# smoggy-P/gym-Drone2D-ActivePerception

Measured on NVIDIA B200. Metric: env-steps/sec, higher is better.
Workload: dtype f64

## Files before the change

### gym_drone2d_activeperception_b200/csrc/d2d_step.cuh

```cuda
#pragma once
#include "d2d_state.cuh"
#include "d2d_math.cuh"
#include "d2d_agent_math.cuh"

#if defined(D2D_COLD_NOINLINE) && D2D_COLD_NOINLINE
#define D2D_COLD __noinline__
#else
#define D2D_COLD __forceinline__
#endif

__device__ __forceinline__ uint32_t d2d_smem_u32(const void *p) { return (uint32_t)__cvta_generic_to_shared(p); }
__device__ __forceinline__ void d2d_mbar_init(uint64_t *bar, uint32_t count) {
    asm volatile("mbarrier.init.shared::cta.b64 [%0], %1;" ::"r"(d2d_smem_u32(bar)), "r"(count) : "memory");
    asm volatile("fence.mbarrier_init.release.cluster;" ::: "memory");
}
__device__ __forceinline__ void d2d_mbar_expect_tx(uint64_t *bar, uint32_t bytes) {
    asm volatile("mbarrier.arrive.expect_tx.shared::cta.b64 _, [%0], %1;" ::"r"(d2d_smem_u32(bar)), "r"(bytes) : "memory");
}
__device__ __forceinline__ void d2d_bulk_g2s(void *dst_smem, const void *src_gmem, uint32_t bytes, uint64_t *bar) {
    asm volatile("cp.async.bulk.shared::cluster.global.mbarrier::complete_tx::bytes [%0], [%1], %2, [%3];" ::"r"(
                     d2d_smem_u32(dst_smem)),
                 "l"(src_gmem), "r"(bytes), "r"(d2d_smem_u32(bar))
                 : "memory");
}
// ... 201 lines not shown
        double vx = pref.x, vy = pref.y;
        const bool rvo = P.motion_rvo != 0;
        if (rvo) {
            const double2 v = P.avel_next[g];
            P.avel[g] = v;
            vx = v.x; vy = v.y;
        }
        const double nx = pos.x + vx * P.dt, ny = pos.y + vy * P.dt;
        bool rebound = false;
        if (d2d_norm2_le(vx, vy, 5.0)) {
            const double qx = D2D_FMA(C6, pref.x, -S6 * pref.y);
            const double qy = D2D_FMA(S6, pref.x, C6 * pref.y);
            pref.x = qx; pref.y = qy;
            rebound = true;
        }
        const double edge = P.scale;
        if (nx < edge + r) pref.x = fabs(pref.x);
        else if (nx > P.map_w - edge - r) pref.x = -fabs(pref.x);
        if (ny < edge + r) pref.y = fabs(pref.y);
        else if (ny > P.map_h - edge - r) pref.y = -fabs(pref.y);
        if (!rebound && !rvo) { vx = pref.x; vy = pref.y; }
        pos.x = pos.x + vx * P.dt;
        pos.y = pos.y + vy * P.dt;
        P.apos[g] = pos;
        P.apref[g] = pref;
        if (PF && keep_pos && w == tid) { *keep_pos = pos; *keep_pref = pref; }
        const int q = i * NP + k;
        c.sx[q] = pos.x; c.sy[q] = pos.y; c.sr2[q] = r * r;
        const double ddx = pos.x - s.px, ddy = pos.y - s.py;
        const double reach = r + P.cull_reach;
        if (ddx * ddx + ddy * ddy <= reach * reach) {
            const int slot = atomicAdd(&s.ncull, 1);
            c.cull[i * NP + slot] = (uint16_t)k;
        }
        if (COLLIDE_HERE) {
            if (d2d_norm2_lt(ddx, ddy, r + P.drone_r)) atomicOr(&s.coll_agent, 1);
        }
    }
}

struct RayOut {
    uint8_t *bel_s;
    int e;
    int patch;
    int wi, wj;
    int border_ok;
    uint32_t *chg;
    int *nchg;
    int defer_mirror;
};
#define D2D_CHG_CAP 64
#define D2D_ACTION_SENTINEL 0x7FF8D2D0AC710F05ull
#define D2D_FUSED_WARP_EXTRA (D2D_CHG_CAP * 4 + 16)

__device__ __forceinline__ void d2d_mark_store(const DevP &P, const RayOut &o, int cell, uint8_t v) {
    o.bel_s[cell] = v;
#if defined(D2D_WARP_PROF) && D2D_WARP_PROF >= 2
    atomicAdd(&P.prof[(size_t)o.e * 12 + 5], 1ull);
#endif
    P.belief[(size_t)o.e * D2D_BELIEF_STRIDE + cell] = v;
    if (o.patch) {
        const int ci = cell / D2D_GRID, cj = cell - ci * D2D_GRID;
        const int u = ci - o.wi, w = cj - o.wj;
        if ((unsigned)u < (unsigned)D2D_LOCAL && (unsigned)w < (unsigned)D2D_LOCAL) {
            const size_t off = (size_t)o.e * D2D_LOCAL_CELLS + u * D2D_LOCAL + w;
            P.local_map[off] = v;
            if (P.lm_mirror && !o.defer_mirror) {
                P.lm_mirror[off] = v;
                atomicAdd((int *)(o.bel_s + D2D_MIRCNT_OFF), 1);
            }
        }
    }
    if (o.chg) {
        const int slot = atomicAdd(o.nchg, 1);
        if (slot < D2D_CHG_CAP) o.chg[slot] = (uint32_t)cell | ((uint32_t)v << 16);
    }
}
__device__ __forceinline__ void d2d_mark(const DevP &P, const RayOut &o, int ci, int cj, uint8_t v) {
    const int cell = ci * D2D_GRID + cj;
    if (o.bel_s[cell] != v) d2d_mark_store(P, o, cell, v);
}

__device__ __forceinline__ double d2d_ray_angle(const DevP &P, double yaw, int ray) {
    const double ray_angle = P.ray_a0 + P.ray_da * (double)ray;
    const double player_angle = D2D_TWO_PI - yaw * D2D_DEG2RAD;
    double a = player_angle + ray_angle;
    a = copysign(d2d_pymod(fabs(a), D2D_TWO_PI), a);
    if (a < 0) a += D2D_TWO_PI;
    return a;
}

template <bool SAFE = false, bool SMALL = false>
__device__ __forceinline__ uint32_t d2d_cast_ray(const DevP &P, const EnvS &s, double a, double slope, const RayOut &o,
                                                 const uint64_t *gt, const double *sx, const double *sy, const double *sr2,
                                                 const uint16_t *cull, uint32_t *hitw) {
    uint32_t hm = 0u;
    const bool faced_right = (a < 90.0 * D2D_DEG2RAD) || (a > 270.0 * D2D_DEG2RAD);
    const bool faced_up = a > D2D_PI;
    const double step = P.scale - 1.0;
    double xs, ys;
    if (fabs(slope) > 1.0) {
        slope = 1.0 / slope;
        ys = faced_up ? -step : step;
        xs = ys * slope;
    } else {
        xs = faced_right ? step : -step;
        ys = xs * slope;
    }
    const double x0 = s.px, y0 = s.py;
    const int nc = s.ncull;
    uint32_t cmask = 0u;
    int mlo = 0x7fff, mhi = -1;
    {
        const double dd2 = xs * xs + ys * ys;
        const float inv_dd2 = 1.0f / (float)dd2;
        const int ncm = (SMALL || nc < 32) ? nc : 32;
#pragma unroll 1
        for (int q = 0; q < ncm; q++) {
            const int k = cull[q];
            const double cx = sx[k] - x0, cy = sy[k] - y0;
            const double cr = cx * ys - cy * xs;
            const double rr = sr2[k] * 1.000001 + 1e-3;
            if (cr * cr <= rr * dd2) {
                cmask |= 1u << q;
                const float t = (float)(cx * xs + cy * ys) * inv_dd2;
                const float hw = sqrtf((float)rr * inv_dd2) + 0.05f;
                mlo = min(mlo, (int)ceilf(t - hw));
                mhi = max(mhi, (int)floorf(t + hw));
            }
        }
        if (!SMALL && nc > 32) { mlo = 0; mhi = 0x7fff; }
    }
    const unsigned mspan = mhi >= mlo ? (unsigned)(mhi - mlo) : 0u;
    if (SAFE) {
        const bool xup = xs > 0.0, yup = ys > 0.0;
        int dcx = xup ? D2D_GRID : -D2D_GRID, dcy = yup ? 1 : -1;
        asm volatile("" : "+r"(dcx), "+r"(dcy));
        const double uxs = fabs(xs), uys = fabs(ys);
        const double ux0 = xup ? x0 : -x0, uy0 = yup ? y0 : -y0;
        double ux = ux0, uy = uy0;
        double uxb = xup ? P.scale * (double)(s.ix + 1) : -(P.scale * (double)s.ix);
        double uyb = yup ? P.scale * (double)(s.iy + 1) : -(P.scale * (double)s.iy);
        const double scale = P.scale;
        const uint32_t bel0 = d2d_smem_u32(o.bel_s);
        uint32_t caddr = bel0 + (uint32_t)(s.ix * D2D_GRID + s.iy);
        int m = 0;
        for (;;) {
            if ((unsigned)(m - mlo) <= mspan) {
                const double x = dcx > 0 ? ux : -ux, y = dcy > 0 ? uy : -uy;
                if (!(0.0 < x && 0.0 < y)) break;
                bool any = false;
                uint32_t mm = cmask;
                while (mm) {
                    const int q = __ffs(mm) - 1;
                    mm &= mm - 1u;
                    const int k = cull[q];
                    const double ex = sx[k] - x, ey = sy[k] - y;
                    if (ex * ex + ey * ey <= sr2[k]) { hm |= 1u << q; any = true; }
                }
                if (!SMALL) {
#pragma unroll 1
                    for (int q = 32; q < nc; q++) {
                        const int k = cull[q];
                        const double ex = sx[k] - x, ey = sy[k] - y;
                        if (ex * ex + ey * ey <= sr2[k]) { atomicOr(&hitw[k >> 5], 1u << (k & 31)); any = true; }
                    }
                }
                if (any) break;
            }
            uint32_t bel;
            asm volatile("ld.shared.u8 %0, [%1];" : "=r"(bel) : "r"(caddr));
            if (bel != 2u) {
                if (bel == 1u) break;
                const int cell = (int)(caddr - bel0);
                const int ci = cell / D2D_GRID, cj = cell - ci * D2D_GRID;
                if ((gt[ci] >> cj) & 1ull) {
                    bool in_map = true;
                    if (ci == 0 || cj == 0) {
                        const double x = dcx > 0 ? ux : -ux, y = dcy > 0 ? uy : -uy;
                        in_map = 0.0 < x && 0.0 < y;
                    }
                    if (in_map) d2d_mark_store(P, o, cell, 1);
                    break;
                }
                if (m >= P.m_far) {
                    const double fx = ux - ux0, fy = uy - uy0;
                    if ((fx * fx + fy * fy) >= P.depth2) break;
                }
                d2d_mark_store(P, o, cell, 2);
            } else if (m >= P.m_far) {
                const double fx = ux - ux0, fy = uy - uy0;
                if ((fx * fx + fy * fy) >= P.depth2) break;
            }
            m += 1;
            asm("{\n\t"
                ".reg .pred pe, pn;\n\t"
                "add.rn.f64 %0, %0, %3;\n\t"
                "setp.lt.s32 pn, %4, 0;\n\t"
                "setp.eq.and.f64 pe, %0, %1, pn;\n\t"
                "setp.lt.or.f64 pe, %0, %1, pe;\n\t"
                "@!pe add.s32 %2, %2, %4;\n\t"
                "@!pe add.rn.f64 %1, %1, %5;\n\t"
                "}" : "+d"(ux), "+d"(uxb), "+r"(caddr) : "d"(uxs), "r"(dcx), "d"(scale));
            asm("{\n\t"
                ".reg .pred pe, pn;\n\t"
                "add.rn.f64 %0, %0, %3;\n\t"
                "setp.lt.s32 pn, %4, 0;\n\t"
                "setp.eq.and.f64 pe, %0, %1, pn;\n\t"
                "setp.lt.or.f64 pe, %0, %1, pe;\n\t"
                "@!pe add.s32 %2, %2, %4;\n\t"
                "@!pe add.rn.f64 %1, %1, %5;\n\t"
                "}" : "+d"(uy), "+d"(uyb), "+r"(caddr) : "d"(uys), "r"(dcy), "d"(scale));
        }
#if defined(D2D_WARP_PROF) && D2D_WARP_PROF >= 2
        atomicAdd(&P.prof[(size_t)o.e * 12 + 6], (unsigned long long)(m + 1));
        atomicMax(&P.prof[(size_t)o.e * 12 + 7], (unsigned long long)(m + 1));
#endif
        return hm;
    }
    int ci = s.ix, cj = s.iy;
    const bool xup = xs > 0.0, yup = ys > 0.0;
    const int sxi = xup ? 1 : -1, syi = yup ? 1 : -1;
    const double uxs = fabs(xs), uys = fabs(ys);
    double ux = xup ? x0 : -x0, uy = yup ? y0 : -y0;
    double uxb = xup ? P.scale * (double)(ci + 1) : -(P.scale * (double)ci);
    double uyb = yup ? P.scale * (double)(cj + 1) : -(P.scale * (double)cj);
    int m = 0;
    for (;;) {
        if ((unsigned)(ci - 1) >= (unsigned)(D2D_GRID - 2) || (unsigned)(cj - 1) >= (unsigned)(D2D_GRID - 2)) {
            const double x = xup ? ux : -ux, y = yup ? uy : -uy;
            if (!(0.0 < x && x < P.map_w && 0.0 < y && y < P.map_h)) break;
        }
        if ((unsigned)(m - mlo) <= mspan) {
            const double x = xup ? ux : -ux, y = yup ? uy : -uy;
            bool any = false;
            uint32_t mm = cmask;
            while (mm) {
                const int q = __ffs(mm) - 1;
                mm &= mm - 1u;
                const int k = cull[q];
                const double ex = sx[k] - x, ey = sy[k] - y;
                if (ex * ex + ey * ey <= sr2[k]) {
                    hm |= 1u << q;
                    any = true;
                }
            }
            if (!SMALL) {
#pragma unroll 1
                for (int q = 32; q < nc; q++) {
                    const int k = cull[q];
                    const double ex = sx[k] - x, ey = sy[k] - y;
                    if (ex * ex + ey * ey <= sr2[k]) {
                        atomicOr(&hitw[k >> 5], 1u << (k & 31));
                        any = true;
                    }
                }
            }
            if (any) break;
        }
        const bool wall = (gt[ci] >> cj) & 1ull;
        bool far = false;
        if (m >= P.m_far) {
            const double fx = ux - (xup ? x0 : -x0), fy = uy - (yup ? y0 : -y0);
            far = (fx * fx + fy * fy) >= P.depth2;
        }
        if (wall || far) {
            if (wall) d2d_mark(P, o, ci, cj, 1);
            break;
        }
        d2d_mark(P, o, ci, cj, 2);
        ux = ux + uxs;
        uy = uy + uys;
        m += 1;
        bool cx = ux >= uxb, cy = uy >= uyb;
        if (ux == uxb || uy == uyb) {
            if (ux == uxb && !xup) cx = false;
            if (uy == uyb && !yup) cy = false;
        }
        if (cx) { ci += sxi; uxb += P.scale; }
        if (cy) { cj += syi; uyb += P.scale; }
    }
    return hm;
}

__device__ __forceinline__ void d2d_publish_hits(uint32_t hm, const uint16_t *cull, uint32_t *hitw) {
    while (hm) {
        const int q = __ffs(hm) - 1;
        hm &= hm - 1u;
        const int k = cull[q];
        atomicOr(&hitw[k >> 5], 1u << (k & 31));
    }
}

__device__ __forceinline__ void d2d_phase_rays(const DevP &P, const BlockCtx &c, int env0, int E, int tid, int T) {
    const int R = P.n_rays, NP = P.NP;
    for (int w = tid; w < E * R; w += T) {
        const int i = w / R, ray = w - i * R;
        const EnvS &s = c.S[i];
        if (!s.valid) continue;
        RayOut o;
        o.bel_s = c.belief + (size_t)i * D2D_BELIEF_STRIDE;
        o.e = env0 + i; o.patch = 0; o.wi = 0; o.wj = 0; o.border_ok = 0; o.chg = nullptr; o.nchg = nullptr; o.defer_mirror = 0;
        const double a = d2d_ray_angle(P, s.yaw, ray);
        const uint32_t hm = d2d_cast_ray(P, s, a, d2d_tan(a), o, c.gt + (size_t)i * D2D_GRID, c.sx + i * NP, c.sy + i * NP,
                                         c.sr2 + i * NP, c.cull + i * NP, c.hitw + i * P.HW);
        d2d_publish_hits(hm, c.cull + i * NP, c.hitw + i * P.HW);
    }
}

__device__ __forceinline__ int d2d_border_intact(const uint64_t *gt, int lane) {
    const uint64_t FULL = (1ull << D2D_GRID) - 1ull, EDGE = 1ull | (1ull << (D2D_GRID - 1));
    bool ok = true;
#pragma unroll
    for (int r = lane; r < D2D_GRID; r += 32) {
        const uint64_t need = (r == 0 || r == D2D_GRID - 1) ? FULL : EDGE;
        ok = ok && ((gt[r] & need) == need);
    }
    return __all_sync(0xffffffffu, ok) ? 1 : 0;
}

template <bool ILP2, bool SMALL = false>
__device__ __forceinline__ uint32_t d2d_phase_rays_warp(const DevP &P, const BlockCtx &c, const RayOut &o, int lane) {
    static_assert(!(ILP2 && SMALL), "the small-crowd form casts one ray per lane per pass");
    const EnvS &s = c.S[0];
    const int R = P.n_rays;
    uint32_t hm = 0u;
    if (ILP2) {
        for (int r0 = lane; r0 < R; r0 += 64) {
            const int r1 = r0 + 32;
            const double a0 = d2d_ray_angle(P, s.yaw, r0), a1 = d2d_ray_angle(P, s.yaw, r1);
            const double t0 = d2d_tan(a0), t1 = d2d_tan(a1);
            hm |= d2d_cast_ray(P, s, a0, t0, o, c.gt, c.sx, c.sy, c.sr2, c.cull, c.hitw);
            if (r1 < R) hm |= d2d_cast_ray(P, s, a1, t1, o, c.gt, c.sx, c.sy, c.sr2, c.cull, c.hitw);
        }
    } else {
        const bool safe = o.border_ok && (unsigned)s.ix < (unsigned)D2D_GRID && (unsigned)s.iy < (unsigned)D2D_GRID;
#pragma unroll 1
        for (int ray = lane; ray < R; ray += 32) {
            const double a = d2d_ray_angle(P, s.yaw, ray);
            const double tn = d2d_tan(a);
            if (safe) hm |= d2d_cast_ray<true, SMALL>(P, s, a, tn, o, c.gt, c.sx, c.sy, c.sr2, c.cull, c.hitw);
            else hm |= d2d_cast_ray<false, SMALL>(P, s, a, tn, o, c.gt, c.sx, c.sy, c.sr2, c.cull, c.hitw);
        }
    }
    hm = __reduce_or_sync(0xffffffffu, hm);
    if (SMALL) return __reduce_or_sync(0xffffffffu, ((hm >> lane) & 1u) ? 1u << c.cull[lane] : 0u);
    if ((hm >> lane) & 1u) {
        const int k = c.cull[lane];
        atomicOr(&c.hitw[k >> 5], 1u << (k & 31));
    }
    return 0u;
}

struct D2DRng {
    uint32_t *key;
    int pos, has;
    double gauss;
};
__device__ __noinline__ void d2d_mt_regen(uint32_t *mt) {
    const uint32_t UP = 0x80000000u, LO = 0x7fffffffu, MA = 0x9908b0dfu;
    int kk;
    uint32_t y;
#pragma unroll 1
    for (kk = 0; kk < 624 - 397; kk++) { y = (mt[kk] & UP) | (mt[kk + 1] & LO); mt[kk] = mt[kk + 397] ^ (y >> 1) ^ ((y & 1u) ? MA : 0u); }
#pragma unroll 1
    for (; kk < 623; kk++) { y = (mt[kk] & UP) | (mt[kk + 1] & LO); mt[kk] = mt[kk + (397 - 624)] ^ (y >> 1) ^ ((y & 1u) ? MA : 0u); }
    y = (mt[623] & UP) | (mt[0] & LO); mt[623] = mt[396] ^ (y >> 1) ^ ((y & 1u) ? MA : 0u);
}
__device__ __forceinline__ uint32_t d2d_mt_next32(D2DRng &r) {
    if (r.pos == 624) { d2d_mt_regen(r.key); r.pos = 0; }
    uint32_t y = r.key[r.pos++];
    y ^= (y >> 11); y ^= (y << 7) & 0x9d2c5680u; y ^= (y << 15) & 0xefc60000u; y ^= (y >> 18);
    return y;
}
__device__ __forceinline__ double d2d_mt_next_double(D2DRng &r) {
    const int a = (int)(d2d_mt_next32(r) >> 5), b = (int)(d2d_mt_next32(r) >> 6);
    return ((double)a * 67108864.0 + (double)b) / 9007199254740992.0;
}
__device__ __noinline__ double d2d_legacy_gauss(D2DRng &r) {
    if (r.has) { const double t = r.gauss; r.has = 0; r.gauss = 0.0; return t; }
    double f, x1, x2, r2;
    do {
        x1 = 2.0 * d2d_mt_next_double(r) - 1.0;
        x2 = 2.0 * d2d_mt_next_double(r) - 1.0;
        r2 = x1 * x1 + x2 * x2;
    } while (r2 >= 1.0 || r2 == 0.0);
// ... 584 lines not shown
        }
        if (lane == 0) atomicAdd(&P.stats[D2D_STAT_MIRROR_BYTES], (unsigned long long)n_changed);
    }
    if (s.done_now) d2d_count_explored_warp(P, c.belief, lane);
    D2D_PROF(3);
}


__device__ __forceinline__ bool d2d_agents_lane(const DevP &P, const BlockCtx &c, EnvS &s, size_t g, int lane, double2 &pos,
                                                double2 &pref, double r) {
    bool in = false, hit = false;
    if (lane < P.N) {
        d2d_cvm_agent_step(pos.x, pos.y, pref.x, pref.y, r, P.dt, P.scale, P.map_w, P.map_h);
        P.apos[g] = pos;
        P.apref[g] = pref;
        c.sx[lane] = pos.x; c.sy[lane] = pos.y; c.sr2[lane] = r * r;
        const double ddx = pos.x - s.px, ddy = pos.y - s.py;
        const double reach = r + P.cull_reach;
        in = ddx * ddx + ddy * ddy <= reach * reach;
        hit = d2d_norm2_lt(ddx, ddy, r + P.drone_r);
    }
    const uint32_t b = __ballot_sync(0xffffffffu, in);
    if (in) c.cull[__popc(b & ((1u << lane) - 1u))] = (uint16_t)lane;
    if (lane == 0) s.ncull = __popc(b);
    return __any_sync(0xffffffffu, hit);
}

__device__ __forceinline__ void d2d_trackers_lane(const DevP &P, const BlockCtx &c, EnvS &s, size_t g, int lane, uint32_t hmask,
                                                  uint8_t pf_act) {
    if (lane >= P.N) return;
    const bool hit = (hmask >> lane) & 1u;
    P.hit[g] = hit ? 1 : 0;
    if (P.trackers) {
        const bool was_active = !s.reset && pf_act != 0;
        if (hit && !was_active) atomicAdd(&s.newly, 1);
        if (was_active || hit || s.reset) {
            const bool noisy = P.var_cam != 0.0;
            d2d_tracker_update(P, s, g, hit, noisy ? c.mx[lane] : c.sx[lane], noisy ? c.my[lane] : c.sy[lane], was_active);
        }
    }
}

__device__ __forceinline__ void d2d_leader_nomove(const DevP &P, EnvS &s, const uint64_t *gt, int e, double action, bool coll,
                                                  int &inv) {
    const int shit = inv & 1;
    bool goal = (inv & 2) != 0;
    s.tgx = -1.0; s.tgy = -1.0;
    if (s.nseg * P.n_way - s.cursor > 0) {
        d2d_leader_finish(P, s, gt, e, 0.0, true, false);
        s.ix = d2d_cell(s.px, P.scale, P.inv_scale); s.iy = d2d_cell(s.py, P.scale, P.inv_scale);
        goal = d2d_norm2_le(s.px - s.tgx, s.py - s.tgy, 10.0);
        int sh = 0;
        for (int q = 0; q < 5; q++) sh |= d2d_static_probe(P, gt, s.px, s.py, q);
        inv = sh | (goal ? 2 : 0);
    } else {
        s.sm = SM_EXECUTING; s.fail = 0;
    }
    s.yaw = d2d_pymod(s.yaw + (action * P.max_yaw_speed) * P.dt, 360.0);
    const int col = shit ? 1 : (coll ? 2 : 0);
    int frz = 0;
    if (col == 0) {
        if (goal) s.sm = SM_GOAL_REACHED;
        frz = ((double)s.steps >= P.max_steps) ? 1 : 0;
    }
    const int done = (col != 0 || frz || (s.sm == SM_GOAL_REACHED && s.tcur >= P.n_targets)) ? 1 : 0;
    s.bufc += s.arch_cnt; s.bufts += s.arch_ts; s.tracked += s.newly;
    if (done) { s.bufc += s.act_cnt; s.bufts += s.act_ts; }
    s.done_now = done;
    P.collision[e] = (uint8_t)col; P.dead_lock[e] = 0; P.freezing[e] = (uint8_t)frz; P.done[e] = (uint8_t)done;
    P.yaw_obs[e] = (float)s.yaw;
    if (P.yaw_mirror) P.yaw_mirror[e] = (float)s.yaw;
    if (P.done_mirror) P.done_mirror[e] = (uint8_t)done;
    if (done) {
        atomicAdd(&P.stats[D2D_STAT_EPISODES], 1ull);
        if (s.sm == SM_GOAL_REACHED) atomicAdd(&P.stats[D2D_STAT_SUCCESS], 1ull);
        if (col == 1) atomicAdd(&P.stats[D2D_STAT_STATIC_COLLISION], 1ull);
        if (col == 2) atomicAdd(&P.stats[D2D_STAT_DYNAMIC_COLLISION], 1ull);
        if (frz) atomicAdd(&P.stats[D2D_STAT_FREEZING], 1ull);
        atomicAdd(&P.stats[D2D_STAT_FLIGHT_STEPS], (unsigned long long)s.steps);
        atomicAdd(&P.stats[D2D_STAT_AGENTS_TRACKED], (unsigned long long)s.bufc);
        atomicAdd(&P.stats[D2D_STAT_TRACKED_STEPS], (unsigned long long)s.bufts);
    }
}

#define D2D_GATE_STAMP_SLOT(B) ((size_t)(B))
#define D2D_SMALL_N 32

template <int WPB, int MINB, bool SYNC, bool GATED, bool SMALL = false>
__global__ void __launch_bounds__(WPB * 32, MINB) d2d_rollout_warp_kernel(const DevP P, const double *__restrict__ actions,
                                                                          int K, long long action_stride, int sync_every,
                                                                          unsigned int t_first) {
    static_assert(!(SMALL && GATED), "the small-crowd form serves d2d_rollout only");
    extern __shared__ __align__(128) unsigned char smem[];
    const int lane = threadIdx.x & 31, wid = threadIdx.x >> 5;
    const int e = blockIdx.x * WPB + wid;
    if (GATED) {
        if (threadIdx.x == 0) *(int *)(smem + (size_t)WPB * d2d_warp_slice_bytes(P.NP, P.HW, D2D_FUSED_WARP_EXTRA)) = 0;
        __syncthreads();
    }
    if (GATED && P.gate_src && blockIdx.x == gridDim.x - 1) {
        unsigned long long &cst = *(unsigned long long *)(smem + (size_t)WPB * d2d_warp_slice_bytes(P.NP, P.HW, D2D_FUSED_WARP_EXTRA) + 128);
        const volatile unsigned long long *hs = (const volatile unsigned long long *)P.gate_stamp_host;
        for (unsigned int t = 0;; t++) {
            if (threadIdx.x == 0) {
                const unsigned long long want = (unsigned long long)(t_first + t);
                const long long t0 = clock64();
                unsigned long long st;
                while ((((st = *hs) >> 1) & 0xffffffffull) != want) {
                    if (clock64() - t0 > 4000000000ll) { *P.gate_fault = 1u; st = (want << 1) | (1ull << 62); break; }
                }
                cst = st;
            }
            __syncthreads();
            const unsigned long long st = cst;
            const bool zero = (st >> 62) & 1ull;
#pragma unroll 1
            for (int i0 = threadIdx.x; i0 < P.B; i0 += 8 * (int)blockDim.x) {
                unsigned long long v[8];
#pragma unroll
                for (int k = 0; k < 8; k++) {
                    const int i = i0 + k * (int)blockDim.x;
                    v[k] = (i < P.B && !zero) ? __ldcv(P.gate_src + i) : 0ull;
                }
#pragma unroll
                for (int k = 0; k < 8; k++) {
                    const int i = i0 + k * (int)blockDim.x;
                    if (i < P.B) P.gate[i] = v[k];
                }
            }
            __syncthreads();
            if (threadIdx.x == 0) {
                __threadfence();
                *(volatile unsigned long long *)(P.gate + D2D_GATE_STAMP_SLOT(P.B)) = st & 0x1ffffffffull;
            }
            if (!(st & 1ull)) return;
        }
    }
    if (e >= P.B) {
        if (SYNC) for (int t = 1; t < K; t++) if (t % sync_every == 0) __syncthreads();
        return;
    }
    unsigned char *slice = smem + (size_t)wid * d2d_warp_slice_bytes(SMALL ? D2D_SMALL_N : P.NP, SMALL ? 1 : P.HW,
                                                                     GATED ? D2D_FUSED_WARP_EXTRA : 0);
    const BlockCtx c = d2d_carve(slice, 1, SMALL ? D2D_SMALL_N : P.NP, SMALL ? 1 : P.HW);
    uint32_t *chg = (uint32_t *)(slice + d2d_step_smem_bytes(1, SMALL ? D2D_SMALL_N : P.NP, SMALL ? 1 : P.HW));
    int *nchg = (int *)(chg + D2D_CHG_CAP);
    unsigned char *blk = smem + (size_t)WPB * d2d_warp_slice_bytes(SMALL ? D2D_SMALL_N : P.NP, SMALL ? 1 : P.HW,
                                                                   GATED ? D2D_FUSED_WARP_EXTRA : 0);
    int *blk_cnt = (int *)blk;
    unsigned int *blk_yaw = (unsigned int *)(blk + 16);
    unsigned int *blk_done = (unsigned int *)(blk + 16 + WPB * 4);
    const int blk_envs = min(WPB, P.B - (int)blockIdx.x * WPB);
    EnvS &s = c.S[0];
    const size_t ga = (size_t)e * P.NP + lane;
    double2 pf_pos = double2{0.0, 0.0}, pf_pref = double2{0.0, 0.0};
    double pf_r = 0.0;
    uint8_t pf_act = 0;
    if (lane < P.N) {
        pf_pos = P.apos[ga]; pf_pref = P.apref[ga]; pf_r = P.arad[ga];
        if (P.trackers) pf_act = P.trk_active[ga];
    }
    double action = GATED ? 0.0 : actions[e];
    if (lane == 0) {
        if (GATED) *nchg = 0;
        d2d_mbar_init(c.mbar, 1);
        d2d_mbar_expect_tx(c.mbar, D2D_GT_ROW_BYTES + D2D_BELIEF_STRIDE);
        d2d_bulk_g2s(c.gt, P.gt_rows + (size_t)e * D2D_GRID, D2D_GT_ROW_BYTES, c.mbar);
        d2d_bulk_g2s(c.belief, P.belief + (size_t)e * D2D_BELIEF_STRIDE, D2D_BELIEF_STRIDE, c.mbar);
        c.misc[0] = 0;
    }
    d2d_load_env_warp(P, s, e, lane);
    if (lane == 0) c.misc[1] = s.reset;
    if (!SMALL) {
#pragma unroll 1
        for (int w = lane; w < P.HW; w += 32) c.hitw[w] = 0u;
    }
    __syncwarp();
    int border_ok = 0;
    const bool mirror = GATED && P.lm_mirror != nullptr;
    int inv = 0;
#pragma unroll 1
    for (int t = 0;;) {
        D2D_PROF(0);
        d2d_reset_prefetch(P, s, e, lane, pf_pos, pf_pref);
        d2d_reset_arrays(P, c, e, 1, lane, 32, t == 0 ? c.mbar : nullptr);
        bool coll = false;
        if (SMALL) coll = d2d_agents_lane(P, c, s, ga, lane, pf_pos, pf_pref, pf_r);
        else d2d_phase_agents<true, true>(P, c, e, 1, lane, 32, pf_pos, pf_pref, pf_r, &pf_pos, &pf_pref);
        if (t == 0 && pf_act && !s.reset) d2d_prefetch_tracker(P, ga);
        if (lane == 0) d2d_leader_begin(P, s);
        __syncwarp();
        if (SMALL) {
            if (t == 0) {
                d2d_mbar_wait(c.mbar, 0);
                border_ok = d2d_border_intact(c.gt, lane);
            }
            if (t == 0 || s.reset) {
                const double px = s.px, py = s.py;
                const int sh = __any_sync(0xffffffffu, lane < 5 ? d2d_static_probe(P, c.gt, px, py, lane) : 0);
                if (lane == 0) {
                    inv = sh | (d2d_norm2_le(px - -1.0, py - -1.0, 10.0) ? 2 : 0);
                    s.ix = d2d_cell(px, P.scale, P.inv_scale); s.iy = d2d_cell(py, P.scale, P.inv_scale);
                }
                __syncwarp();
            }
        }
        const bool refill = s.reset && s.obs_ix == s.ix && s.obs_iy == s.iy && (GATED || P.lm_mirror == nullptr);
        const bool patch = (!s.reset || refill) && s.obs_ix == s.ix && s.obs_iy == s.iy;
        if (refill) d2d_obs_clear_warp(P, e, lane, false);
        RayOut ro;
        ro.bel_s = c.belief; ro.e = e; ro.patch = patch ? 1 : 0;
        ro.wi = s.ix - 16; ro.wj = s.iy - 16;
        ro.chg = (mirror && patch && !refill) ? chg : nullptr; ro.nchg = nchg; ro.defer_mirror = GATED ? 1 : 0;
        if (!SMALL && t == 0) {
            d2d_mbar_wait(c.mbar, 0);
            border_ok = d2d_border_intact(c.gt, lane);
        }
        ro.border_ok = border_ok;
        D2D_PROF(1);
        const uint32_t hmask = d2d_phase_rays_warp<false, SMALL>(P, c, ro, lane);
        __syncwarp();
        D2D_PROF(2);
        if (P.var_cam != 0.0) {
            if (lane == 0) {
                if (SMALL) c.hitw[0] = hmask;
                d2d_measure_env(P, c, e);
            }
            __syncwarp();
        }
        if (SMALL) d2d_trackers_lane(P, c, s, ga, lane, hmask, pf_act);
        else d2d_phase_trackers<true>(P, c, e, 1, lane, 32, pf_act);
        const int shit = SMALL ? 0 : __any_sync(0xffffffffu, lane < 5 ? d2d_static_probe(P, c.gt, s.px, s.py, lane) : 0);
        __syncwarp();
        int more = (t + 1 < K) ? 1 : 0;
        bool rewrite = false;
        int n_changed = 0;
        if (GATED) {
            if (lane == 0) {
                s.tgx = -1.0; s.tgy = -1.0;
                d2d_leader_finish(P, s, c.gt, e, 0.0, true, false);
                d2d_leader_flags(P, s, c.gt, e, shit, false);
            }
            __syncwarp();
            n_changed = (mirror && !refill) ? *nchg : 0;
            rewrite = !patch || s.ix != s.obs_ix || s.iy != s.obs_iy || (mirror && n_changed > D2D_CHG_CAP);
            __syncwarp();
            if (rewrite && lane == 0) { s.obs_ix = s.ix; s.obs_iy = s.iy; }
            __syncwarp();
            if (rewrite) d2d_obs_env_warp(P, c.belief, s.ix, s.iy, e, lane, false);
            if (s.done_now) d2d_count_explored_warp(P, c.belief, lane);
            D2D_PROF(8);
            if (lane == 0) {
                volatile unsigned long long *slot = P.gate + e;
                volatile unsigned long long *stamp = P.gate + D2D_GATE_STAMP_SLOT(P.B);
                const unsigned long long want = (unsigned long long)(t_first + (unsigned int)t);
                const long long t0 = clock64();
                unsigned long long bits, st = 0ull;
// ... 106 lines not shown
```

### gym_drone2d_activeperception_b200/csrc/drone2d.cu

```cuda
#include <cstddef>
#include <cstdio>
#include <cstdlib>
#include <cstring>
#include <cmath>
#include <string>
#include <vector>
#include <initializer_list>

#include "d2d_state.cuh"
#include "d2d_math.cuh"
#include "d2d_step.cuh"
#include "d2d_plan.cuh"
#include "d2d_rvo.cuh"
#include "d2d_clone.cuh"
#include "d2d_worldgen.cuh"
#include "d2d_episode.cuh"
#include "d2d_render.cuh"
#include "d2d_difficulty.cuh"

struct EnvRows {
    int64_t row_bytes, row_stride;
    int planes;
    int64_t plane_stride;
};
// ... 914 lines not shown
    }
    const int epb = h->cfg.envs_per_block;
    if (h->cfg.planner == D2D_PLANNER_NOMOVE && epb <= 0) {
        rc = launch_fused_warp<4, 7, false>(h, actions_dev, st);
    } else if (h->cfg.planner == D2D_PLANNER_NOMOVE && epb == 1) {
        rc = launch_fused_warp<4, 7, true>(h, actions_dev, st);
    } else if (h->cfg.planner == D2D_PLANNER_NOMOVE && epb == 2) {
        rc = launch_fused_warp<4, 7, false>(h, actions_dev, st);
    } else if (h->cfg.planner == D2D_PLANNER_NOMOVE && epb == 3) {
        rc = launch_fused_warp<7, 4, true>(h, actions_dev, st);
    } else if (h->cfg.planner == D2D_PLANNER_NOMOVE) {
        switch (h->E) {
            case 4: rc = launch_fused<4>(h, actions_dev, st); break;
            case 16: rc = launch_fused<16>(h, actions_dev, st); break;
            default: rc = launch_fused<8>(h, actions_dev, st); break;
        }
    } else if (h->cfg.planner == D2D_PLANNER_JERK) {
        if (!h->jerk_set) { h->err = "planner = Jerk_Primitive: d2d_set_jerk_tables must provide the heading tables"; return D2D_ERR_STATE; }
        rc = launch_jerk_warp<4>(h, actions_dev, st);
    } else {
        rc = step_primitive(h, actions_dev, st);
    }
    if (rc != D2D_OK) return rc;
    CUDA_TRY(h, cudaGetLastError());
    return D2D_OK;
}

static int launch_prim_warp_entry(d2d_handle *h, const double *actions, cudaStream_t st, double *ox_next);

extern "C" int d2d_step_plan_oxford(d2d_handle *h, const double *actions_dev, double *next_actions_dev, void *stream) {
    if (!h || !actions_dev || !next_actions_dev) return D2D_ERR_INVALID;
    D2D_NO_PIPE(h);
    if (!h->world_set) { h->err = "d2d_step_plan_oxford before d2d_set_world"; return D2D_ERR_STATE; }
    if (!(h->cfg.oxford & D2D_POLICY_OXFORD)) { h->err = "d2d_step_plan_oxford: handle was created without the Oxford state (cfg.oxford & 1)"; return D2D_ERR_STATE; }
    if (h->cfg.var_cam != 0.0 && !h->rng_set) { h->err = "var_cam != 0: d2d_set_rng must provide the np.random stream state"; return D2D_ERR_STATE; }
    if (h->cfg.planner != D2D_PLANNER_PRIMITIVE || h->cfg.envs_per_block > 0 || h->P.motion_rvo) {
        int rc = step_impl(h, actions_dev, stream);
        if (rc == D2D_OK) rc = d2d_plan_oxford(h, next_actions_dev, stream);
        return rc != D2D_OK ? rc : log_step(h, (cudaStream_t)stream);
    }
    CUDA_TRY(h, cudaSetDevice(h->cfg.device));
    const int rc = launch_prim_warp_entry(h, actions_dev, (cudaStream_t)stream, next_actions_dev);
    if (rc != D2D_OK) return rc;
    CUDA_TRY(h, cudaGetLastError());
    return log_step(h, (cudaStream_t)stream);
}

#define D2D_RESIDENT_WPB 28

template <int WPB, int MINB, bool SYNC, bool GATED, bool SMALL = false>
static int launch_rollout(d2d_handle *h, const double *actions, int K, long long stride, cudaStream_t st, unsigned int t_first = 0,
                          int extra_blocks = 0) {
    const size_t smem = (size_t)WPB * d2d_warp_slice_bytes(SMALL ? D2D_SMALL_N : h->NP, SMALL ? 1 : h->HW,
                                                           GATED ? D2D_FUSED_WARP_EXTRA : 0) + (GATED ? 256 : 0);
    if (smem > 227 * 1024) { h->err = "rollout kernel: shared memory per block exceeds 227 KB"; return D2D_ERR_INVALID; }
    const int rc = ensure_smem_attr(h, (const void *)d2d_rollout_warp_kernel<WPB, MINB, SYNC, GATED, SMALL>, "rollout warp");
    if (rc != D2D_OK) return rc;
    static const int sync_every = getenv("D2D_ROLLOUT_SYNC") ? atoi(getenv("D2D_ROLLOUT_SYNC")) : 1;
    d2d_rollout_warp_kernel<WPB, MINB, SYNC, GATED, SMALL><<<(h->B + WPB - 1) / WPB + extra_blocks, WPB * 32, smem, st>>>(
        h->P, actions, K, stride, sync_every > 0 ? sync_every : 1, t_first);
    return D2D_OK;
}

static int resident_capacity(d2d_handle *h) {
    if (h->resident_capacity >= 0) return h->resident_capacity;
    constexpr int WPB = D2D_RESIDENT_WPB;
    const size_t smem = (size_t)WPB * d2d_warp_slice_bytes(h->NP, h->HW, D2D_FUSED_WARP_EXTRA) + 256;
    int cap = 0, nb = 0, sms = 0;
    if (smem <= 227 * 1024 && ensure_smem_attr(h, (const void *)d2d_rollout_warp_kernel<WPB, 1, false, true>, "rollout warp") == D2D_OK &&
        cudaOccupancyMaxActiveBlocksPerMultiprocessor(&nb, d2d_rollout_warp_kernel<WPB, 1, false, true>, WPB * 32, smem) == cudaSuccess &&
        cudaDeviceGetAttribute(&sms, cudaDevAttrMultiProcessorCount, h->cfg.device) == cudaSuccess)
        { cap = nb * sms * WPB; h->resident_blocks = nb * sms; }
    else
        cudaGetLastError();
    if (getenv("D2D_PIPE_DEBUG")) fprintf(stderr, "[d2d pipelined] resident kernel: %d blocks/SM x %d SMs, smem %zu B -> capacity %d envs (%s)\n", nb, sms, smem, cap, cudaGetErrorString(cudaPeekAtLastError()));
    h->resident_capacity = cap;
    return cap;
}

extern "C" int d2d_rollout(d2d_handle *h, const double *actions_dev, int32_t num_steps, int64_t action_stride, void *stream) {
    if (!h || !actions_dev || num_steps < 1) return D2D_ERR_INVALID;
    D2D_NO_PIPE(h);
    if (!h->world_set) { h->err = "d2d_rollout before d2d_set_world"; return D2D_ERR_STATE; }
    if (h->cfg.var_cam != 0.0 && !h->rng_set) { h->err = "var_cam != 0: d2d_set_rng must provide the np.random stream state"; return D2D_ERR_STATE; }
    if (h->cfg.planner != D2D_PLANNER_NOMOVE || h->P.motion_rvo || h->cfg.envs_per_block > 0) {
        h->err = "d2d_rollout: NoMove planner, CVM motion profile and the default warp kernels only (use d2d_step)";
        return D2D_ERR_INVALID;
    }
    if (action_stride != 0 && action_stride < h->B) { h->err = "d2d_rollout: action_stride must be 0 or >= num_envs"; return D2D_ERR_INVALID; }
    CUDA_TRY(h, cudaSetDevice(h->cfg.device));
    cudaStream_t st = (cudaStream_t)stream;
    static const int variant = getenv("D2D_ROLLOUT_VARIANT") ? atoi(getenv("D2D_ROLLOUT_VARIANT")) : 0;
    int rc;
    if ((variant == 0 && h->B > 2 * 28 * 148) || h->ep_mem) {
        for (int t = 0; t < num_steps; t++) {
            rc = launch_fused_warp<4, 7, false>(h, actions_dev + (size_t)t * (size_t)action_stride, st);
            if (rc == D2D_OK) rc = log_step(h, st);
            if (rc != D2D_OK) return rc;
        }
        CUDA_TRY(h, cudaGetLastError());
        return D2D_OK;
    }
    switch (variant) {
        case 1: rc = launch_rollout<4, 7, false, false>(h, actions_dev, num_steps, action_stride, st); break;
        case 2: rc = launch_rollout<4, 7, true, false>(h, actions_dev, num_steps, action_stride, st); break;
        case 3: rc = launch_rollout<7, 4, true, false>(h, actions_dev, num_steps, action_stride, st); break;
        case 4: rc = launch_rollout<14, 2, true, false>(h, actions_dev, num_steps, action_stride, st); break;
// ... 751 lines not shown
```

Baseline: 243.6 million.

## Skip rays in angular sectors with no unexplored cells or nearby obstacles

Adds a per-warp angular sector bitmap for the small-crowd rollout path. Each cell in a box around the drone gets an angular span code, and a difference array counts unexplored cells per 64-sector ring. Marking a cell decrements its sectors, and moving obstacles within reach also set their sectors live. Rays whose angle falls in a dead sector are compacted out, so only live rays are cast. This removes redundant ray casting when the nearby map is already explored. In exchange it adds shared memory per warp, sector init on every move, and atomic bookkeeping on each mark, and it relies on conservative margins to stay exact.

```diff
diff --git a/gym_drone2d_activeperception_b200/csrc/d2d_step.cuh b/gym_drone2d_activeperception_b200/csrc/d2d_step.cuh
--- a/gym_drone2d_activeperception_b200/csrc/d2d_step.cuh
+++ b/gym_drone2d_activeperception_b200/csrc/d2d_step.cuh
@@ -277,8 +277,43 @@
 #define D2D_CHG_CAP 64
 #define D2D_ACTION_SENTINEL 0x7FF8D2D0AC710F05ull
 #define D2D_FUSED_WARP_EXTRA (D2D_CHG_CAP * 4 + 16)
-
+#define D2D_SMALL_N 32
+
+#define D2D_SEC 64
+#define D2D_SEC_H 10
+#define D2D_SEC_BOX (2 * D2D_SEC_H + 1)
+#define D2D_SEC_WORDS ((D2D_SEC_BOX * D2D_SEC_BOX + 31) / 32)
+#define D2D_SEC_DIFFALL_OFF (D2D_SEC * 4)
+#define D2D_SEC_LIST_OFF (D2D_SEC_DIFFALL_OFF + D2D_SEC * 4)
+#define D2D_SEC_OUT_OFF (D2D_SEC_LIST_OFF + 64)
+#define D2D_SEC_OUTALL_OFF (D2D_SEC_OUT_OFF + 64)
+#define D2D_SEC_POSE_OFF (D2D_SEC_OUTALL_OFF + 64)
+#define D2D_SEC_CODES_OFF (D2D_SEC_POSE_OFF + 16)
+#define D2D_SKIP_BYTES (D2D_SEC_CODES_OFF + (D2D_SEC_BOX * D2D_SEC_BOX * 2 + 15) / 16 * 16)
+__device__ __forceinline__ unsigned char *d2d_sec_base(uint8_t *bel_s) {
+    return bel_s + d2d_step_smem_bytes(1, D2D_SMALL_N, 1);
+}
+__device__ __forceinline__ void d2d_sec_add(int *diff, uint32_t code, int d) {
+    const int lo = (int)(code & 63u), end = lo + (int)((code >> 6) & 63u) + 1;
+    atomicAdd(&diff[lo], d);
+    if (end < D2D_SEC) atomicAdd(&diff[end], -d);
+    else if (end > D2D_SEC) { atomicAdd(&diff[0], d); atomicAdd(&diff[end - D2D_SEC], -d); }
+}
+__device__ __forceinline__ void d2d_sec_unmark(uint8_t *bel_s, int wi, int wj, int cell) {
+    const int ci = cell / D2D_GRID, cj = cell - ci * D2D_GRID;
+    const int u = ci - wi - (16 - D2D_SEC_H), w = cj - wj - (16 - D2D_SEC_H);
+    if ((unsigned)u < (unsigned)D2D_SEC_BOX && (unsigned)w < (unsigned)D2D_SEC_BOX) {
+        unsigned char *sec = d2d_sec_base(bel_s);
+        const int q = u * D2D_SEC_BOX + w;
+        const uint32_t bit = 1u << (q & 31);
+        if (!(atomicOr((uint32_t *)(sec + D2D_SEC_OUT_OFF) + (q >> 5), bit) & bit))
+            d2d_sec_add((int *)sec, ((const uint16_t *)(sec + D2D_SEC_CODES_OFF))[q], -1);
+    }
+}
+
+template <bool SEC = false>
 __device__ __forceinline__ void d2d_mark_store(const DevP &P, const RayOut &o, int cell, uint8_t v) {
+    if (SEC) d2d_sec_unmark(o.bel_s, o.wi, o.wj, cell);
     o.bel_s[cell] = v;
 #if defined(D2D_WARP_PROF) && D2D_WARP_PROF >= 2
     atomicAdd(&P.prof[(size_t)o.e * 12 + 5], 1ull);
@@ -301,9 +336,10 @@
         if (slot < D2D_CHG_CAP) o.chg[slot] = (uint32_t)cell | ((uint32_t)v << 16);
     }
 }
+template <bool SEC = false>
 __device__ __forceinline__ void d2d_mark(const DevP &P, const RayOut &o, int ci, int cj, uint8_t v) {
     const int cell = ci * D2D_GRID + cj;
-    if (o.bel_s[cell] != v) d2d_mark_store(P, o, cell, v);
+    if (o.bel_s[cell] != v) d2d_mark_store<SEC>(P, o, cell, v);
 }
 
 __device__ __forceinline__ double d2d_ray_angle(const DevP &P, double yaw, int ray) {
@@ -405,14 +441,14 @@
                         const double x = dcx > 0 ? ux : -ux, y = dcy > 0 ? uy : -uy;
                         in_map = 0.0 < x && 0.0 < y;
                     }
-                    if (in_map) d2d_mark_store(P, o, cell, 1);
+                    if (in_map) d2d_mark_store<SMALL>(P, o, cell, 1);
                     break;
                 }
                 if (m >= P.m_far) {
                     const double fx = ux - ux0, fy = uy - uy0;
                     if ((fx * fx + fy * fy) >= P.depth2) break;
                 }
-                d2d_mark_store(P, o, cell, 2);
+                d2d_mark_store<SMALL>(P, o, cell, 2);
             } else if (m >= P.m_far) {
                 const double fx = ux - ux0, fy = uy - uy0;
                 if ((fx * fx + fy * fy) >= P.depth2) break;
@@ -490,10 +526,10 @@
             far = (fx * fx + fy * fy) >= P.depth2;
         }
         if (wall || far) {
-            if (wall) d2d_mark(P, o, ci, cj, 1);
+            if (wall) d2d_mark<SMALL>(P, o, ci, cj, 1);
             break;
         }
-        d2d_mark(P, o, ci, cj, 2);
+        d2d_mark<SMALL>(P, o, ci, cj, 2);
         ux = ux + uxs;
         uy = uy + uys;
         m += 1;
@@ -544,6 +580,134 @@
     return __all_sync(0xffffffffu, ok) ? 1 : 0;
 }
 
+#define D2D_SEC_MARGIN 1e-4f
+#define D2D_SEC_K 10.185916357881302f
+
+__device__ __forceinline__ uint32_t d2d_sec_code(float lo, float width) {
+    const int s0 = (int)floorf((lo - D2D_SEC_MARGIN) * D2D_SEC_K);
+    const int s1 = (int)floorf((lo + width + D2D_SEC_MARGIN) * D2D_SEC_K);
+    const int span = s1 - s0;
+    if (span >= D2D_SEC - 1) return 0x8000u | (63u << 6);
+    return 0x8000u | ((uint32_t)span << 6) | (uint32_t)(s0 & (D2D_SEC - 1));
+}
+__device__ __forceinline__ unsigned long long d2d_sec_bits(uint32_t code) {
+    const int lo = (int)(code & 63u), span = (int)((code >> 6) & 63u);
+    if (span == 63) return ~0ull;
+    const unsigned long long m = (2ull << span) - 1ull;
+    return lo ? (m << lo) | (m >> (64 - lo)) : m;
+}
+
+__device__ __forceinline__ uint32_t d2d_sec_cell(const DevP &P, double px, double py, int ci, int cj, bool own, bool wall) {
+    if (own) return 0x8000u | (63u << 6);
+    const double x0 = P.scale * (double)ci, x1 = x0 + P.scale, y0 = P.scale * (double)cj, y1 = y0 + P.scale;
+    const double dx = px < x0 ? x0 - px : (px > x1 ? px - x1 : 0.0);
+    const double dy = py < y0 ? y0 - py : (py > y1 ? py - y1 : 0.0);
+    if (wall) {
+        if (dx * dx + dy * dy >= P.cull_reach * P.cull_reach) return 0u;
+    } else {
+        const double xx = __dmul_rn(dx, dx), yy = __dmul_rn(dy, dy);
+        const double d2 = fmin(__dadd_rn(xx, yy), fmin(__fma_rn(dx, dx, yy), __fma_rn(dy, dy, xx)));
+        if (!(d2 < P.depth2)) return 0u;
+    }
+    const double g = 1e-3;
+    const int xs = px < x0 - g ? 1 : (px > x1 + g ? -1 : 0);
+    const int ys = py < y0 - g ? 1 : (py > y1 + g ? -1 : 0);
+    if (xs == 0 && ys == 0) {
+        const int nx = px < x0 + g ? 1 : (px > x1 - g ? -1 : 0), ny = py < y0 + g ? 1 : (py > y1 - g ? -1 : 0);
+        if (nx == 0 && ny == 0) return 0x8000u | (63u << 6);
+        const float c = atan2f((float)ny, (float)nx), hw = (nx && ny) ? 0.78539816f : 1.5707964f;
+        return d2d_sec_code(c - hw, 2.0f * hw);
+    }
+    const double gx0 = x0 - g - px, gx1 = x1 + g - px, gy0 = y0 - g - py, gy1 = y1 + g - py;
+    double ax, ay, bx, by;
+    if (xs == 0) { ay = by = ys > 0 ? gy0 : gy1; ax = gx0; bx = gx1; }
+    else if (ys == 0) { ax = bx = xs > 0 ? gx0 : gx1; ay = gy0; by = gy1; }
+    else if (xs == ys) { ax = gx1; ay = gy0; bx = gx0; by = gy1; }
+    else { ax = gx0; ay = gy0; bx = gx1; by = gy1; }
+    const float ta = atan2f((float)ay, (float)ax), tb = atan2f((float)by, (float)bx);
+    float d = tb - ta;
+    if (d > 3.14159265f) d -= 6.28318531f;
+    else if (d < -3.14159265f) d += 6.28318531f;
+    return d < 0.0f ? d2d_sec_code(tb, -d) : d2d_sec_code(ta, d);
+}
+
+__device__ __forceinline__ void d2d_sec_init(const DevP &P, const BlockCtx &c, const EnvS &s, int lane, bool full) {
+    unsigned char *sec = d2d_sec_base(c.belief);
+    int *diff = (int *)sec, *diff_all = (int *)(sec + D2D_SEC_DIFFALL_OFF);
+    uint32_t *out = (uint32_t *)(sec + D2D_SEC_OUT_OFF), *out_all = (uint32_t *)(sec + D2D_SEC_OUTALL_OFF);
+    if (!full) {
+        diff[lane] = diff_all[lane]; diff[lane + 32] = diff_all[lane + 32];
+        if (lane < D2D_SEC_WORDS) out[lane] = out_all[lane];
+        __syncwarp();
+        return;
+    }
+    uint16_t *codes = (uint16_t *)(sec + D2D_SEC_CODES_OFF);
+    diff[lane] = 0; diff[lane + 32] = 0; diff_all[lane] = 0; diff_all[lane + 32] = 0;
+    __syncwarp();
+    const double px = s.px, py = s.py;
+    const int ix = s.ix, iy = s.iy;
+#pragma unroll 1
+    for (int k = 0; k < D2D_SEC_WORDS; k++) {
+        const int q = 32 * k + lane;
+        uint32_t code = 0u;
+        bool explored = true;
+        if (q < D2D_SEC_BOX * D2D_SEC_BOX) {
+            const int u = q / D2D_SEC_BOX, w = q - u * D2D_SEC_BOX;
+            const int ci = ix - D2D_SEC_H + u, cj = iy - D2D_SEC_H + w;
+            if ((unsigned)ci < (unsigned)D2D_GRID && (unsigned)cj < (unsigned)D2D_GRID) {
+                code = d2d_sec_cell(P, px, py, ci, cj, ci == ix && cj == iy, (c.gt[ci] >> cj) & 1ull);
+                explored = c.belief[ci * D2D_GRID + cj] != 0;
+            }
+            codes[q] = (uint16_t)code;
+        }
+        if (code) {
+            d2d_sec_add(diff_all, code, 1);
+            if (!explored) d2d_sec_add(diff, code, 1);
+        }
+        const uint32_t z = __ballot_sync(0xffffffffu, code == 0u), zo = __ballot_sync(0xffffffffu, code == 0u || explored);
+        if (lane == 0) { out_all[k] = z; out[k] = zo; }
+    }
+    if (lane == 0) { ((double *)(sec + D2D_SEC_POSE_OFF))[0] = px; ((double *)(sec + D2D_SEC_POSE_OFF))[1] = py; }
+    __syncwarp();
+}
+
+__device__ __forceinline__ unsigned long long d2d_sec_live(const BlockCtx &c, const EnvS &s, int lane) {
+    const int *diff = (const int *)d2d_sec_base(c.belief);
+    int lo = diff[lane], hi = diff[lane + 32];
+#pragma unroll
+    for (int o = 1; o < 32; o <<= 1) {
+        const int a = __shfl_up_sync(0xffffffffu, lo, o), b = __shfl_up_sync(0xffffffffu, hi, o);
+        if (lane >= o) { lo += a; hi += b; }
+    }
+    hi += __shfl_sync(0xffffffffu, lo, 31);
+    unsigned long long live = (unsigned long long)__ballot_sync(0xffffffffu, lo != 0) |
+                              ((unsigned long long)__ballot_sync(0xffffffffu, hi != 0) << 32);
+    if (s.ncull) {
+        unsigned long long m = 0ull;
+        if (lane < s.ncull) {
+            const int k = c.cull[lane];
+            const float dx = (float)(c.sx[k] - s.px), dy = (float)(c.sy[k] - s.py);
+            const float rs = sqrtf((float)c.sr2[k]) * 1.0001f + 1e-2f;
+            const float d2 = dx * dx + dy * dy;
+            if (d2 <= rs * rs) m = ~0ull;
+            else {
+                const float h = asinf(fminf(1.0f, rs * rsqrtf(d2))) + D2D_SEC_MARGIN;
+                m = d2d_sec_bits(d2d_sec_code(atan2f(dy, dx) - h, 2.0f * h));
+            }
+        }
+        live |= (unsigned long long)__reduce_or_sync(0xffffffffu, (unsigned)m) |
+                ((unsigned long long)__reduce_or_sync(0xffffffffu, (unsigned)(m >> 32)) << 32);
+    }
+    return live;
+}
+
+__device__ __forceinline__ bool d2d_ray_live(const DevP &P, double yaw, int ray, unsigned long long live) {
+    const float a = (float)((D2D_TWO_PI - yaw * D2D_DEG2RAD) + (P.ray_a0 + P.ray_da * (double)ray));
+    const int s0 = (int)floorf((a - D2D_SEC_MARGIN) * D2D_SEC_K) & (D2D_SEC - 1);
+    const int s1 = (int)floorf((a + D2D_SEC_MARGIN) * D2D_SEC_K) & (D2D_SEC - 1);
+    return (((live >> s0) | (live >> s1)) & 1ull) != 0ull;
+}
+
 template <bool ILP2, bool SMALL = false>
 __device__ __forceinline__ uint32_t d2d_phase_rays_warp(const DevP &P, const BlockCtx &c, const RayOut &o, int lane) {
     static_assert(!(ILP2 && SMALL), "the small-crowd form casts one ray per lane per pass");
@@ -557,6 +721,31 @@
             const double t0 = d2d_tan(a0), t1 = d2d_tan(a1);
             hm |= d2d_cast_ray(P, s, a0, t0, o, c.gt, c.sx, c.sy, c.sr2, c.cull, c.hitw);
             if (r1 < R) hm |= d2d_cast_ray(P, s, a1, t1, o, c.gt, c.sx, c.sy, c.sr2, c.cull, c.hitw);
+        }
+    } else if (SMALL) {
+        const bool safe = o.border_ok && (unsigned)s.ix < (unsigned)D2D_GRID && (unsigned)s.iy < (unsigned)D2D_GRID;
+        const bool skip = P.lm_mirror == nullptr && P.cull_reach < (double)D2D_SEC_H * P.scale;
+        const unsigned long long live = skip ? d2d_sec_live(c, s, lane) : ~0ull;
+        uint8_t *list = d2d_sec_base(o.bel_s) + D2D_SEC_LIST_OFF;
+        const uint32_t lt = (1u << lane) - 1u;
+#pragma unroll 1
+        for (int r0 = 0; r0 < R; r0 += 64) {
+            const int ra = r0 + lane, rb = r0 + 32 + lane;
+            const uint32_t b0 = __ballot_sync(0xffffffffu, ra < R && d2d_ray_live(P, s.yaw, ra, live));
+            const uint32_t b1 = __ballot_sync(0xffffffffu, rb < R && d2d_ray_live(P, s.yaw, rb, live));
+            const int n0 = __popc(b0), n = n0 + __popc(b1);
+            if ((b0 >> lane) & 1u) list[__popc(b0 & lt)] = (uint8_t)lane;
+            if ((b1 >> lane) & 1u) list[n0 + __popc(b1 & lt)] = (uint8_t)(32 + lane);
+            __syncwarp();
+#pragma unroll 1
+            for (int i = lane; i < n; i += 32) {
+                const int ray = r0 + list[i];
+                const double a = d2d_ray_angle(P, s.yaw, ray);
+                const double tn = d2d_tan(a);
+                if (safe) hm |= d2d_cast_ray<true, true>(P, s, a, tn, o, c.gt, c.sx, c.sy, c.sr2, c.cull, c.hitw);
+                else hm |= d2d_cast_ray<false, true>(P, s, a, tn, o, c.gt, c.sx, c.sy, c.sr2, c.cull, c.hitw);
+            }
+            __syncwarp();
         }
     } else {
         const bool safe = o.border_ok && (unsigned)s.ix < (unsigned)D2D_GRID && (unsigned)s.iy < (unsigned)D2D_GRID;
@@ -1247,7 +1436,7 @@
         goal = d2d_norm2_le(s.px - s.tgx, s.py - s.tgy, 10.0);
         int sh = 0;
         for (int q = 0; q < 5; q++) sh |= d2d_static_probe(P, gt, s.px, s.py, q);
-        inv = sh | (goal ? 2 : 0);
+        inv = sh | (goal ? 2 : 0) | 4;
     } else {
         s.sm = SM_EXECUTING; s.fail = 0;
     }
@@ -1279,7 +1468,6 @@
 }
 
 #define D2D_GATE_STAMP_SLOT(B) ((size_t)(B))
-#define D2D_SMALL_N 32
 
 template <int WPB, int MINB, bool SYNC, bool GATED, bool SMALL = false>
 __global__ void __launch_bounds__(WPB * 32, MINB) d2d_rollout_warp_kernel(const DevP P, const double *__restrict__ actions,
@@ -1336,12 +1524,12 @@
         return;
     }
     unsigned char *slice = smem + (size_t)wid * d2d_warp_slice_bytes(SMALL ? D2D_SMALL_N : P.NP, SMALL ? 1 : P.HW,
-                                                                     GATED ? D2D_FUSED_WARP_EXTRA : 0);
+                                                                     GATED ? D2D_FUSED_WARP_EXTRA : (SMALL ? D2D_SKIP_BYTES : 0));
     const BlockCtx c = d2d_carve(slice, 1, SMALL ? D2D_SMALL_N : P.NP, SMALL ? 1 : P.HW);
     uint32_t *chg = (uint32_t *)(slice + d2d_step_smem_bytes(1, SMALL ? D2D_SMALL_N : P.NP, SMALL ? 1 : P.HW));
     int *nchg = (int *)(chg + D2D_CHG_CAP);
     unsigned char *blk = smem + (size_t)WPB * d2d_warp_slice_bytes(SMALL ? D2D_SMALL_N : P.NP, SMALL ? 1 : P.HW,
-                                                                   GATED ? D2D_FUSED_WARP_EXTRA : 0);
+                                                                   GATED ? D2D_FUSED_WARP_EXTRA : (SMALL ? D2D_SKIP_BYTES : 0));
     int *blk_cnt = (int *)blk;
     unsigned int *blk_yaw = (unsigned int *)(blk + 16);
     unsigned int *blk_done = (unsigned int *)(blk + 16 + WPB * 4);
@@ -1390,6 +1578,7 @@
                 d2d_mbar_wait(c.mbar, 0);
                 border_ok = d2d_border_intact(c.gt, lane);
             }
+            const bool moved = t == 0 || (__shfl_sync(0xffffffffu, inv, 0) & 4);
             if (t == 0 || s.reset) {
                 const double px = s.px, py = s.py;
                 const int sh = __any_sync(0xffffffffu, lane < 5 ? d2d_static_probe(P, c.gt, px, py, lane) : 0);
@@ -1398,6 +1587,11 @@
                     s.ix = d2d_cell(px, P.scale, P.inv_scale); s.iy = d2d_cell(py, P.scale, P.inv_scale);
                 }
                 __syncwarp();
+            }
+            if (moved || s.reset) {
+                const double *cp = (const double *)(d2d_sec_base(c.belief) + D2D_SEC_POSE_OFF);
+                d2d_sec_init(P, c, s, lane, moved || cp[0] != s.px || cp[1] != s.py);
+                if (lane == 0) inv &= ~4;
             }
         }
         const bool refill = s.reset && s.obs_ix == s.ix && s.obs_iy == s.iy && (GATED || P.lm_mirror == nullptr);
diff --git a/gym_drone2d_activeperception_b200/csrc/drone2d.cu b/gym_drone2d_activeperception_b200/csrc/drone2d.cu
--- a/gym_drone2d_activeperception_b200/csrc/drone2d.cu
+++ b/gym_drone2d_activeperception_b200/csrc/drone2d.cu
@@ -990,7 +990,8 @@
 static int launch_rollout(d2d_handle *h, const double *actions, int K, long long stride, cudaStream_t st, unsigned int t_first = 0,
                           int extra_blocks = 0) {
     const size_t smem = (size_t)WPB * d2d_warp_slice_bytes(SMALL ? D2D_SMALL_N : h->NP, SMALL ? 1 : h->HW,
-                                                           GATED ? D2D_FUSED_WARP_EXTRA : 0) + (GATED ? 256 : 0);
+                                                           GATED ? D2D_FUSED_WARP_EXTRA : (SMALL ? D2D_SKIP_BYTES : 0)) +
+                        (GATED ? 256 : 0);
     if (smem > 227 * 1024) { h->err = "rollout kernel: shared memory per block exceeds 227 KB"; return D2D_ERR_INVALID; }
     const int rc = ensure_smem_attr(h, (const void *)d2d_rollout_warp_kernel<WPB, MINB, SYNC, GATED, SMALL>, "rollout warp");
     if (rc != D2D_OK) return rc;
```

Result: slower. 237.8 million (median of 6 runs) (-2.4%).
